# johannes-graeter/limo

Measured on NVIDIA H100. Metric: BA windows/s (30 KF, 3k LM, 40k obs), higher is better.
Workload: dtype f64

## Files before the change

### limo_b200/csrc/kba_api.cu

```cuda
#include <algorithm>
#include <atomic>
#include <chrono>
#include <cstdio>
#include <cstdlib>
#include <cstring>
#include <string>
#include <thread>
#include <vector>

#include <cuda_runtime.h>

#include "kba_b200.h"
#include "kba_kernels.h"

using namespace kba;

static thread_local std::string g_last_error;
static thread_local bool g_force_host_pack = false;
static int fail(int code, const std::string& msg) {
    g_last_error = msg;
    return code;
}
#define CU(call)                                                                                              \
    do {                                                                                                      \
// ... 603 lines not shown
        int max_chunks = 1;
        for (auto& d : b->desc_h) max_chunks = std::max(max_chunks, d.n_chunks);
        int p = std::min(16, (6 * h->sm_count + n_windows * pairs - 1) / (n_windows * pairs));
        b->lc.small_syrk = (max_rows <= 184);
        if (b->lc.small_syrk) p = (h->sm_count + n_windows - 1) / n_windows;
        bd.p_split = std::max(1, std::min(p, max_chunks));
        const char* fe = std::getenv("KBA_FUSED");
        bd.fused = (b->lc.small_syrk && bd.max_kf <= kFusedMaxKf && !(fe && std::atoi(fe) == 0)) ? 1 : 0;
        if (const char* pe = std::getenv("KBA_P_SPLIT")) { if (std::atoi(pe) > 0) p = std::atoi(pe); }
        if (bd.fused) bd.p_split = std::max(1, std::min(p, max_groups));
        else if (std::getenv("KBA_P_SPLIT")) bd.p_split = std::max(1, std::min(p, max_chunks));
        b->lc.fused_slots = (max_rows_free <= 176) ? 6 : 7;
    }
    bd.cost_parts = std::max((bd.max_obs + 255) / 256, (bd.max_obs / 16 + bd.max_lm / 32 + 4 + 7) / 8);
    { const char* le = std::getenv("KBA_LINEARIZE"); b->lc.lin_fused = !(le && std::atoi(le) == 0); }
    { const char* le = std::getenv("KBA_LIN_BLOCKS"); if (le && std::atoi(le) == 3) b->lc.lin_blocks = 3; }
    { const char* le = std::getenv("KBA_LIN_GRID"); if (le) b->lc.lin_grid = std::max(-1, std::atoi(le)); }
    { const char* le = std::getenv("KBA_BS_GRID"); if (le) b->lc.bs_grid = std::max(-1, std::atoi(le)); }
    {
        auto knob = [](const char* name, int dflt) { const char* e = std::getenv(name); return e ? std::atoi(e) : dflt; };
        bd.eval_tiles_jac = std::max(1, knob("KBA_EVAL_TILES_JAC", 8));
        bd.eval_tiles_cost = std::max(1, knob("KBA_EVAL_TILES_COST", 8));
        bd.eval_min_blocks = knob("KBA_EVAL_MIN_BLOCKS", 2);
        bd.eval_cs = knob("KBA_EVAL_CS", 0);
        bd.solve_row_major = knob("KBA_SOLVE_ROW_MAJOR", 0);
        bd.solve_tiled = (nr_cap_max <= 192 && !bd.solve_row_major) ? 1 : 0;
        const int split_dflt = (!bd.solve_tiled && n_windows <= 16) ? std::max(1, std::min(32, h->sm_count / n_windows)) : 0;
        bd.solve_split = bd.solve_tiled ? 0 : knob("KBA_SOLVE_SPLIT", split_dflt);
    }
    bd.bs_parts = (bd.max_lm + 15) / 16;
    {
// ... 242 lines not shown
    launch_reset(b->bd, lc, s);
    const int rounds_max = 7;
    const int max_passes = rounds_max * (3 * opt->trim_solver_iterations + 4) + opt->final_solver_iterations + 8;
    const auto t0 = std::chrono::steady_clock::now();
    int check_every = 4;
    bool timed_out = false, poll_pending = false;
    int gmode = solve_graph_mode();
    if (h->kernel_timing || launch_check_enabled() || s == nullptr || b->sg.unusable) gmode = 0;
    const bool lockstep = b->bd.sharded != 0;
    if (lockstep) gmode = (gmode && shard_graph_enabled() && b->solves_done > 0) ? 1 : 0;
    if (gmode) {
        std::vector<unsigned char> key;
        key.reserve(sizeof(BatchDev) + sizeof(SolveParams) + 64);
        key_append(key, b->bd); key_append(key, sp); key_append(key, gmode); key_append(key, max_passes); key_append(key, s);
        key_append(key, lc.nr_cap_max); key_append(key, lc.max_rank); key_append(key, (int)lc.small_syrk); key_append(key, (int)lc.lin_fused);
        key_append(key, lc.lin_blocks); key_append(key, lc.fused_slots); key_append(key, lc.xchg.user);
        key_append(key, lc.lin_grid); key_append(key, lc.bs_grid);
        if (!(b->sg.exec && b->sg.key == key) && !build_solve_graph(b, sp, lc, gmode, max_passes, check_every, key)) gmode = 0;
    }
    if (gmode == 2) {
        CU(cudaMemsetAsync(b->loop_pass.d, 0, sizeof(int), s));
        CU(cudaGraphLaunch(b->sg.exec, s));
        CU(b->loop_pass.download(s));
        CU(cudaEventRecord(b->ev_b, s));
        CU(b->jac_obs.download(s));
        CU(wait_stream(h));
        CU(cudaGetLastError());
        CU(cudaEventElapsedTime(&b->last_solve_ms, b->ev_a, b->ev_b));
        h->counters.jacobian_obs += (long long)b->jac_obs.h[0];
        add_pass_counters(h->counters, b->sg.per_pass, b->loop_pass.h[0]);
        h->counters.launches_total += b->loop_pass.h[0];
// ... 531 lines not shown
```

### limo_b200/csrc/kba_device.cuh

```cuda
#pragma once
#include <cstdint>
#include <cuda_runtime.h>

namespace kba {

constexpr int kMaxKf = 128;
constexpr int kMaxCam = 8;
constexpr int kPoseStride = 12;
constexpr int kCamStride = 16;
constexpr int kIterLogCap = 160;
constexpr int kFusedMaxKf = 32;

struct WinDesc {
    int n_kf, n_cam, n_lm, n_obs, n_gp;
    int kf_off, cam_off, lm_off, obs_off, gp_off;
    int chunk_off, n_chunks;
    int grp_off, n_groups;
    int scale_kf0, scale_kf1;
    double scale_weight, scale_value;
    double plane_reg_weight;
    int plane_dist_fixed, landmarks_fixed;
    int speed_kf, pad0;
    double speed_weight, speed_dt;
    double speed_v_before[3];
// ... 191 lines not shown
        o[2] = q0 * p[2] - q1 * p[3] + q2 * p[0] + q3 * p[1];
        o[3] = q0 * p[3] + q1 * p[2] - q2 * p[1] + q3 * p[0];
    } else {
        o[0] = p[0]; o[1] = p[1]; o[2] = p[2]; o[3] = p[3];
    }
    o[4] = p[4] + d[3]; o[5] = p[5] + d[4]; o[6] = p[6] + d[5];
}

template <typename T, bool kCost = true>
__device__ inline void cauchy(T b, T w, T s, T& half_rho, T& sqrt_rho1) {
    const T sum = T(1) + s / b;
    half_rho = kCost ? T(0.5) * w * b * log(sum) : T(0);
    sqrt_rho1 = sqrt(w / sum);
}

template <typename T, bool kJac, bool kCost = true>
__device__ inline bool eval_observation(const T* __restrict__ pose, const T* __restrict__ cam, const T p[3], T u, T v,
                                        T d, T wt, T b_repr, T b_depth, T r[3], T jp[18], T jl[9], T& half_rho_sum,
                                        T raw[2]) {
    const T a0 = pose[0] * p[0] + pose[1] * p[1] + pose[2] * p[2];
    const T a1 = pose[3] * p[0] + pose[4] * p[1] + pose[5] * p[2];
    const T a2 = pose[6] * p[0] + pose[7] * p[1] + pose[8] * p[2];
    const T x0 = a0 + pose[9], x1 = a1 + pose[10], x2 = a2 + pose[11];
    const T c0 = cam[0] * x0 + cam[1] * x1 + cam[2] * x2 + cam[9];
    const T c1 = cam[3] * x0 + cam[4] * x1 + cam[5] * x2 + cam[10];
    const T c2 = cam[6] * x0 + cam[7] * x1 + cam[8] * x2 + cam[11];
    if (!(fabs(c2) >= T(0.01))) return false;
    const T f = cam[12], iz = T(1) / c2;
    const T xn = c0 * iz, yn = c1 * iz;
    const T ru = f * xn + cam[13] - u, rv = f * yn + cam[14] - v;
    const T s = ru * ru + rv * rv;
    T hr, sq;
    cauchy<T, kCost>(b_repr, wt, s, hr, sq);
    half_rho_sum = hr;
    raw[0] = sqrt(s);
    raw[1] = T(-1);
    r[0] = sq * ru; r[1] = sq * rv; r[2] = T(0);
    T sqd = T(0), rd = T(0);
    const bool has_d = d > T(0);
    if (has_d) {
        rd = c2 - d;
        T hrd;
        cauchy<T, kCost>(b_depth, wt, rd * rd, hrd, sqd);
        half_rho_sum += hrd;
        raw[1] = fabs(rd);
        r[2] = sqd * rd;
    }
    if (kJac) {
        const T fz = f * iz * sq;
        T m[3][3];
#pragma unroll
        for (int c = 0; c < 3; ++c) {
            m[0][c] = fz * (cam[c] - xn * cam[6 + c]);
            m[1][c] = fz * (cam[3 + c] - yn * cam[6 + c]);
            m[2][c] = sqd * cam[6 + c];
        }
#pragma unroll
        for (int i = 0; i < 3; ++i) {
            jp[6 * i + 0] = T(-2) * (m[i][1] * a2 - m[i][2] * a1);
            jp[6 * i + 1] = T(-2) * (m[i][2] * a0 - m[i][0] * a2);
            jp[6 * i + 2] = T(-2) * (m[i][0] * a1 - m[i][1] * a0);
            jp[6 * i + 3] = m[i][0];
            jp[6 * i + 4] = m[i][1];
            jp[6 * i + 5] = m[i][2];
#pragma unroll
            for (int c = 0; c < 3; ++c) jl[3 * i + c] = m[i][0] * pose[c] + m[i][1] * pose[3 + c] + m[i][2] * pose[6 + c];
        }
    }
    return true;
}

template <typename T, bool kCs>
__device__ __forceinline__ void lin_store(T* p, T v) {
    if (kCs) __stcs(p, v); else *p = v;
}
template <typename T, bool kJl = true, bool kCs = false>
__device__ inline bool eval_observation_store(const T* __restrict__ pose, const T* __restrict__ cam, const T p[3], T u,
                                              T v, T d, T wt, T b_repr, T b_depth, T* __restrict__ res,
                                              T* __restrict__ jp, T* __restrict__ jl, size_t stride, bool write_jp,
                                              T& half_rho_sum) {
    const T a0 = pose[0] * p[0] + pose[1] * p[1] + pose[2] * p[2];
// ... 127 lines not shown
```

### limo_b200/csrc/kba_kernels.cu

```cuda
#include "kba_device.cuh"
#include "kba_kernels.h"
#include "kba_regularisers.cuh"
#include "kba_prep.cuh"
#include "kba_linearize.cuh"

#include <cfloat>
#include <cstdio>
#include <cstdlib>
#include <cmath>
#include <type_traits>

namespace kba {

constexpr int kBeginThreads = 1024;
__global__ void __launch_bounds__(kBeginThreads) k_solve_begin(BatchDev bd, SolveParams sp) {
    const int w = blockIdx.x;
    WinState& st = bd.state[w];
    if (st.phase != PH_SOLVE_BEGIN) return;
    const WinDesc wd = bd.desc[w];
    __shared__ int s_has[kMaxKf];
    __shared__ int s_plane[kMaxKf];
    __shared__ int s_cnt[3];
    __shared__ int s_tile_chunk[513];
    for (int k = threadIdx.x; k < wd.n_kf; k += blockDim.x) { s_has[k] = 0; s_plane[k] = 0; }
// ... 365 lines not shown
        (kJac ? bd.gp_cost_x : bd.gp_cost_c)[w] = s;
    }
}
template __global__ void k_gp_eval<true>(BatchDev, SolveParams);
template __global__ void k_gp_eval<false>(BatchDev, SolveParams);

__global__ void __launch_bounds__(256, 2) k_pose_hessian(BatchDev bd, SolveParams sp) {
    const int w = blockIdx.y, k = blockIdx.x;
    const WinState& st = bd.state[w];
    if (st.phase != PH_ITERATE || !st.need_linearize) return;
    const WinDesc& wd = bd.desc[w];
    if (k >= wd.n_kf || bd.off_pose[wd.kf_off + k] < 0) return;
    __shared__ double s_pose[kPoseStride];
    __shared__ double s_cam[kMaxCam * kCamStride];
    __shared__ double s_red[8][27];
    if (threadIdx.x == 0) {
        const double* p = bd.pose[st.cur] + 7 * (size_t)(wd.kf_off + k);
        double R[9];
        quat_to_rot<double>(p, R);
        for (int i = 0; i < 9; ++i) s_pose[i] = R[i];
        s_pose[9] = p[4]; s_pose[10] = p[5]; s_pose[11] = p[6];
    }
    for (int i = threadIdx.x; i < wd.n_cam * kCamStride; i += blockDim.x) s_cam[i] = bd.cam[(size_t)wd.cam_off * kCamStride + i];
    __syncthreads();
    double acc[27];
#pragma unroll
    for (int q = 0; q < 27; ++q) acc[q] = 0.0;
    const int* kp = bd.kf_ptr + wd.kf_off + w;
    const int e0 = kp[k], e1 = kp[k + 1];
    const double* __restrict__ lm_buf = bd.lm[st.cur];
    const size_t ob = (size_t)wd.obs_off;
    int e = e0 + threadIdx.x;
    int idx_b = (e < e1) ? bd.pm_lm[ob + e] : -1;
    int idx_a = (e + (int)blockDim.x < e1) ? bd.pm_lm[ob + e + blockDim.x] : -1;
    int L = -1, cam = 0;
    float u = 0.f, v = 0.f, d = 0.f;
    double p0 = 0, p1 = 0, p2 = 0, wgt = 0;
    unsigned char act = 0;
    if (idx_b >= 0) {
        L = wd.lm_off + idx_b;
        cam = bd.pm_cam[ob + e]; u = bd.pm_u[ob + e]; v = bd.pm_v[ob + e]; d = bd.pm_d[ob + e];
        p0 = lm_buf[3 * (size_t)L]; p1 = lm_buf[3 * (size_t)L + 1]; p2 = lm_buf[3 * (size_t)L + 2];
        wgt = bd.lm_weight[L]; act = bd.lm_active[L];
    }
#pragma unroll 1
    for (; e < e1; e += blockDim.x) {
        const int en = e + blockDim.x;
        int Ln = -1, camn = 0;
        float un = 0.f, vn = 0.f, dn = 0.f;
        double q0 = 0, q1 = 0, q2 = 0, wn = 0;
        unsigned char actn = 0;
        if (idx_a >= 0) {
            Ln = wd.lm_off + idx_a;
            camn = bd.pm_cam[ob + en]; un = bd.pm_u[ob + en]; vn = bd.pm_v[ob + en]; dn = bd.pm_d[ob + en];
            q0 = lm_buf[3 * (size_t)Ln]; q1 = lm_buf[3 * (size_t)Ln + 1]; q2 = lm_buf[3 * (size_t)Ln + 2];
            wn = bd.lm_weight[Ln]; actn = bd.lm_active[Ln];
        }
        idx_a = (en + (int)blockDim.x < e1) ? bd.pm_lm[ob + en + blockDim.x] : -1;
        if (act) {
            const double p[3] = {p0, p1, p2};
            double r[3], jp[18], jl[9], raw[2], hr;
            if (eval_observation<double, true, false>(s_pose, s_cam + kCamStride * cam, p, (double)u, (double)v, (double)d,
                                                      wgt, sp.reprojection_thres * sp.reprojection_thres,
                                                      sp.depth_thres * sp.depth_thres, r, jp, jl, hr, raw)) {
                int q = 0;
#pragma unroll
                for (int a = 0; a < 6; ++a)
#pragma unroll
                    for (int b = a; b < 6; ++b) {
                        acc[q] += jp[a] * jp[b] + jp[6 + a] * jp[6 + b] + jp[12 + a] * jp[12 + b];
                        ++q;
                    }
#pragma unroll
                for (int a = 0; a < 6; ++a) acc[21 + a] += jp[a] * r[0] + jp[6 + a] * r[1] + jp[12 + a] * r[2];
            }
        }
        L = Ln; cam = camn; u = un; v = vn; d = dn; p0 = q0; p1 = q1; p2 = q2; wgt = wn; act = actn;
    }
#pragma unroll
    for (int q = 0; q < 27; ++q) {
        const double v = warp_sum(acc[q]);
        if ((threadIdx.x & 31) == 0) s_red[threadIdx.x >> 5][q] = v;
    }
    __syncthreads();
    if (threadIdx.x < 27) {
        double s = 0.0;
        for (int q = 0; q < 8; ++q) s += s_red[q][threadIdx.x];
        bd.bkf[(size_t)(wd.kf_off + k) * 27 + threadIdx.x] = s;
    }
}

constexpr int kLC = 32;
constexpr int kKC = 3 * kLC;

__device__ __forceinline__ int gp_row(const BatchDev& bd, const WinDesc& wd, int k, int r) {
    if (r < 6) { const int o = bd.off_pose[wd.kf_off + k]; return o < 0 ? -1 : o + r; }
// ... 1591 lines not shown
        e = cudaFuncSetAttribute(k_reduced_solve<true>, cudaFuncAttributeMaxDynamicSharedMemorySize,
                                 (int)solve_tiled_smem(nr_cap_max));
        if (e != cudaSuccess) return e;
        hi_tiled[dev] = nr_cap_max;
    }
    if (nr_cap_max > hi_rows[dev]) {
        e = cudaFuncSetAttribute(k_chol_trail, cudaFuncAttributeMaxDynamicSharedMemorySize, (int)trail_smem(nr_cap_max));
        if (e != cudaSuccess) return e;
        e = cudaFuncSetAttribute(k_reduced_solve<false>, cudaFuncAttributeMaxDynamicSharedMemorySize, (int)solve_smem(nr_cap_max));
        if (e != cudaSuccess) return e;
        hi_rows[dev] = nr_cap_max;
    }
    return cudaSuccess;
}

static int strided_grid(int cfg, int n_units, int num, int den, int n_win, int sm_count) {
    if (cfg == 0) return n_units;
    if (cfg > 0) return cfg < n_units ? cfg : n_units;
    const int g = (n_units * num + den - 1) / den;
    return ((long long)g * n_win >= 8LL * 2 * sm_count && g >= 1) ? g : n_units;
}

void launch_reset(const BatchDev& bd, const LaunchCfg& lc, cudaStream_t s) {
    k_reset_state<<<bd.n_win, 256, 0, s>>>(bd, lc.rounds_override, lc.min_landmarks_for_trimming, lc.num_rounds_option); LCHK("k_reset_state");
}

int launch_pass(const BatchDev& bd, const SolveParams& sp, const LaunchCfg& lc, Counters* cnt, cudaStream_t s) {
    const int B = bd.n_win;
    const dim3 g_obs((bd.max_obs + 255) / 256, B);
    const dim3 g_lm((bd.max_lm + 63) / 64, B);
    if (!bd.fused) k_panel_zero<<<dim3(64, B), 256, 0, s>>>(bd);
    LCHK("k_panel_zero");
    k_solve_begin<<<B, kBeginThreads, 0, s>>>(bd, sp); LCHK("k_solve_begin");
    const bool timed = lc.time_jacobian && lc.ev_pool && *lc.ev_used + 2 <= lc.ev_cap;
    const bool lin1 = bd.lin1 != 0;
    if (lin1) {
        if (bd.tot_gp > 0) k_gp_eval<true><<<B, 256, 0, s>>>(bd, sp);
        LCHK("k_gp_eval");
        if (timed) cudaEventRecord(lc.ev_pool[(*lc.ev_used)++], s);
        const int n_units = (lin_tile_bound(bd.max_obs, bd.max_lm) + kLinWarps - 1) / kLinWarps;
        const dim3 g_lin(strided_grid(lc.lin_grid, n_units, 1, 5, B, lc.sm_count), B);
        if ((int)g_lin.x < n_units) k_linearize<2, true><<<g_lin, kLinThreads, 0, s>>>(bd, sp, n_units);
        else if (lc.lin_blocks == 3) k_linearize<3, false><<<g_lin, kLinThreads, 0, s>>>(bd, sp, n_units);
        else k_linearize<2, false><<<g_lin, kLinThreads, 0, s>>>(bd, sp, n_units);
        LCHK("k_linearize");
        if (timed) cudaEventRecord(lc.ev_pool[(*lc.ev_used)++], s);
        k_pose_hessian<<<dim3(bd.max_kf, B), 256, 0, s>>>(bd, sp); LCHK("k_pose_hessian");
    } else {
        if (timed) cudaEventRecord(lc.ev_pool[(*lc.ev_used)++], s);
        launch_eval_obs<true>(bd, sp, s);
        if (timed) cudaEventRecord(lc.ev_pool[(*lc.ev_used)++], s);
        if (bd.tot_gp > 0) k_gp_eval<true><<<B, 256, 0, s>>>(bd, sp);
        LCHK("k_gp_eval");
        k_pose_hessian<<<dim3(bd.max_kf, B), 256, 0, s>>>(bd, sp); LCHK("k_pose_hessian");
    }
    if (bd.fused) {
        if (!lin1) {
            k_landmark_reduce<true><<<dim3((bd.max_lm + 15) / 16, B), 256, 0, s>>>(bd, sp); LCHK("k_landmark_reduce");
            k_obs_v2<<<g_obs, 256, 0, s>>>(bd); LCHK("k_obs_v2");
// ... 35 lines not shown
        k_reduced_solve<true><<<B, 512, solve_tiled_smem(lc.nr_cap_max), s>>>(bc, sp, 0); LCHK("k_reduced_solve");
    } else if (!bd.solve_split) {
        k_reduced_solve<false><<<B, 512, solve_smem(lc.nr_cap_max), s>>>(bc, sp, 0); LCHK("k_reduced_solve");
    } else {
        k_reduced_solve<false><<<B, 512, solve_smem(lc.nr_cap_max), s>>>(bc, sp, 1); LCHK("k_reduced_solve");
        const int strips = (lc.nr_cap_max + 7) / 8;
        for (int kb = 0; kb < lc.nr_cap_max; kb += kNB) {
            k_chol_diag<<<B, 32, 0, s>>>(bc, kb); LCHK("k_chol_diag");
            k_chol_panel<<<dim3((strips + 15) / 16, B), 512, 0, s>>>(bc, kb); LCHK("k_chol_panel");
            k_chol_trail<<<dim3(bd.solve_split, B), 512, trail_smem(lc.nr_cap_max), s>>>(bc, kb); LCHK("k_chol_trail");
        }
        k_reduced_solve<false><<<B, 512, solve_smem(lc.nr_cap_max), s>>>(bc, sp, 2); LCHK("k_reduced_solve");
    }
    if (bd.fused) {
        const int n_units = (bd.max_lm + 15) / 16;
        const int gx = strided_grid(lc.bs_grid, n_units, 1, 3, B, lc.sm_count);
        if (gx < n_units) k_backsub_v<true><<<dim3(gx, B), 256, 0, s>>>(bd, n_units);
        else k_backsub_v<false><<<dim3(n_units, B), 256, 0, s>>>(bd, n_units);
    }
    else k_backsub<<<dim3((bd.max_lm + 15) / 16, B), 256, 0, s>>>(bd);
    LCHK("k_backsub");
    launch_eval_obs<false>(bd, sp, s);
    if (bd.tot_gp > 0) k_gp_eval<false><<<B, 256, 0, s>>>(bd, sp);
    LCHK("k_gp_eval");
    if (bd.sharded) {
        k_shard_scalars<<<1, 256, 0, s>>>(bd); LCHK("k_shard_scalars");
        if (int rc = lc.xchg.allreduce(lc.xchg.user, bd.xs, bd.xs, 16 + bd.shard_world, 0, s)) return rc;
    }
    k_lm_update<<<(B * 32 + 127) / 128, 128, 0, s>>>(bd, sp); LCHK("k_lm_update");
    k_trim_eval<<<g_lm, 256, 0, s>>>(bd, sp); LCHK("k_trim_eval");
    if (bd.sharded) {
// ... 71 lines not shown
```

### limo_b200/csrc/kba_kernels.h

```cpp
#pragma once
#include <cuda_runtime.h>

#include "kba_device.cuh"

namespace kba {

int launch_check_enabled();
void launch_check_report(const char* kernel, cudaError_t e);
#define LCHK(name)                                                                       \
    do {                                                                                 \
        if (kba::launch_check_enabled()) {                                               \
            const cudaError_t lchk_e_ = cudaGetLastError();                              \
            if (lchk_e_ != cudaSuccess) kba::launch_check_report(name, lchk_e_);         \
        }                                                                                \
    } while (0)

struct Counters {
    long long launches_total = 0;
    long long launches_jacobian = 0, launches_prep = 0, launches_schur = 0, launches_solve = 0, launches_backsub = 0,
              launches_cost = 0, launches_update = 0, launches_trim = 0;
    double ms_jacobian = 0.0;
    long long jacobian_obs = 0;
};

struct Exchange {
    int (*allreduce)(void* user, const double* send, double* recv, long long count, int op, cudaStream_t s) = nullptr;
    void* user = nullptr;
    int rank = 0, world = 1;
};

struct LaunchCfg {
    int nr_cap_max = 64;
    int sm_count = 132;
    int max_rank = 0;
    bool small_syrk = false;
    bool lin_fused = true;
    int lin_blocks = 2;
    int lin_grid = -1;
    int bs_grid = -1;
    int fused_slots = 6;
    int rounds_override = -1, min_landmarks_for_trimming = 100, num_rounds_option = 1;
    bool time_jacobian = false;
    cudaEvent_t* ev_pool = nullptr;
    int ev_cap = 0;
    int* ev_used = nullptr;
    Exchange xchg;
    struct WinDescHost { int nr_cap = 0, n_kf = 0; } shard_win;
};

struct PackRaw {
    const int* lm_ptr = nullptr;
    const int* obs_kf = nullptr;
// ... 51 lines not shown
```

### limo_b200/csrc/kba_linearize.cuh

```cuda
#pragma once
#include "kba_device.cuh"

namespace kba {

constexpr int kLinThreads = 256;
constexpr int kLinWarps = kLinThreads / 32;

__host__ __device__ __forceinline__ int lin_tile_bound(int n_obs, int n_lm) { return n_obs / 16 + n_lm / 32 + 4; }
__device__ __forceinline__ size_t lin_tile_offset(const WinDesc& wd, int w) {
    return (size_t)(wd.obs_off / 16) + (size_t)(wd.lm_off / 32) + 4 * (size_t)w;
}

__device__ inline void build_lin_tiles(const BatchDev& bd, const WinDesc& wd, WinState& st, int w, int* s_chunk ) {
    const int* lm_ptr = bd.lm_ptr + wd.lm_off + w;
    int2* tiles = bd.lin_tile + lin_tile_offset(wd, w);
    const int per = max(64, (wd.n_lm + 511) / 512);
    const int n_chunks = (wd.n_lm + per - 1) / per;
    for (int pass = 0; pass < 2; ++pass) {
        for (int c = threadIdx.x; c < n_chunks; c += blockDim.x) {
            const int j0 = c * per, j1 = min(wd.n_lm, j0 + per);
            int n = 0, t_start = 0, t_cnt = 0;
            int2* out = tiles + (pass ? s_chunk[c] : 0);
            int o0 = lm_ptr[j0];
            for (int j = j0; j < j1; ++j) {
// ... 11 lines not shown
        __syncthreads();
        if (!pass) {
            if (threadIdx.x == 0) {
                int acc = 0;
                for (int c = 0; c < n_chunks; ++c) { const int t = s_chunk[c]; s_chunk[c] = acc; acc += t; }
                if (acc > lin_tile_bound(wd.n_obs, wd.n_lm)) acc = 0;
                st.n_lin_tiles = acc;
                s_chunk[512] = acc;
            }
            __syncthreads();
            if (s_chunk[512] == 0) return;
        }
    }
}

template <int kMinBlocks, bool kLoop>
__global__ void __launch_bounds__(kLinThreads, kMinBlocks) k_linearize(BatchDev bd, SolveParams sp, int n_units) {
    const int w = blockIdx.y;
    WinState& st = bd.state[w];
    if (st.phase != PH_ITERATE) return;
    const WinDesc& wd = bd.desc[w];
    const int n_tiles = st.n_lin_tiles;
    const bool lin = st.need_linearize != 0;
    const bool want_cost = lin && st.iter0;
    if (wd.landmarks_fixed && !want_cost) return;
    const int tid = threadIdx.x, lane = tid & 31, warp = tid >> 5;
    __shared__ __align__(16) double s_pose[kFusedMaxKf * kPoseStride];
    __shared__ __align__(16) double s_cam[kMaxCam * kCamStride];
    __shared__ __align__(8) uint64_t s_bar;
    __shared__ double s_cg[kLinWarps][9][33];
    __shared__ double s_red[kLinWarps];
    __shared__ int s_cnt[kLinWarps];
    bool staged = false;
    for (int unit = blockIdx.x; unit < n_units; unit += gridDim.x) {
    if (unit * kLinWarps >= n_tiles) {
        if (tid == 0 && want_cost) bd.cost_part_x[(size_t)w * bd.cost_parts + unit] = 0.0;
        if constexpr (!kLoop) return;
        continue;
    }
    const size_t base = (size_t)wd.obs_off;
    const int* lm_ptr = bd.lm_ptr + wd.lm_off + w;
    const int t = unit * kLinWarps + warp;
    int2 tile = make_int2(0, 0);
    if (t < n_tiles) tile = bd.lin_tile[lin_tile_offset(wd, w) + t];
    const bool have = lane < tile.y;
    const int o = tile.x + lane;
    int j = 0, kf = 0, cam = 0, row0 = -1, p0 = 0, p1 = 0;
    float mu = 0.f, mv = 0.f, md = 0.f;
    double p[3] = {0, 0, 0}, wgt = 0.0;
    bool act = false;
    if (have) {
        const size_t oo = base + o;
        j = bd.obs_lm[oo];
        kf = bd.obs_kf[oo]; cam = bd.obs_cam[oo]; row0 = bd.obs_row[oo];
        mu = bd.obs_u[oo]; mv = bd.obs_v[oo]; md = bd.obs_d[oo];
        p0 = lm_ptr[j]; p1 = lm_ptr[j + 1];
        act = bd.lm_active[wd.lm_off + j] != 0;
        const double* lmp = bd.lm[st.cur] + 3 * (size_t)(wd.lm_off + j);
        p[0] = lmp[0]; p[1] = lmp[1]; p[2] = lmp[2];
        wgt = bd.lm_weight[wd.lm_off + j];
    }
    const int L = wd.lm_off + j;
    if (!staged) {
        stage_window_bulk(wd, bd.rt[st.cur], bd.cam, s_pose, s_cam, &s_bar);
        staged = true;
    }
    double jp[18];
    bool ok = true;
    double hr = 0.0;
    double cg[9] = {0, 0, 0, 0, 0, 0, 0, 0, 0};
    if (act) {
        double r[3], jl[9], raw[2];
        const double* ps = s_pose + kPoseStride * kf;
        const double* cs_ = s_cam + kCamStride * cam;
        const double br = sp.reprojection_thres * sp.reprojection_thres, bdp = sp.depth_thres * sp.depth_thres;
        if (want_cost) ok = eval_observation<double, true, true>(ps, cs_, p, (double)mu, (double)mv, (double)md, wgt, br, bdp, r, jp, jl, hr, raw);
        else ok = eval_observation<double, true, false>(ps, cs_, p, (double)mu, (double)mv, (double)md, wgt, br, bdp, r, jp, jl, hr, raw);
        if (ok) {
            cg[0] = jl[0] * jl[0] + jl[3] * jl[3] + jl[6] * jl[6];
            cg[1] = jl[0] * jl[1] + jl[3] * jl[4] + jl[6] * jl[7];
            cg[2] = jl[0] * jl[2] + jl[3] * jl[5] + jl[6] * jl[8];
            cg[3] = jl[1] * jl[1] + jl[4] * jl[4] + jl[7] * jl[7];
            cg[4] = jl[1] * jl[2] + jl[4] * jl[5] + jl[7] * jl[8];
            cg[5] = jl[2] * jl[2] + jl[5] * jl[5] + jl[8] * jl[8];
#pragma unroll
            for (int c = 0; c < 3; ++c) cg[6 + c] = jl[c] * r[0] + jl[3 + c] * r[1] + jl[6 + c] * r[2];
        } else {
            hr = 0.0;
            if (lin) st.eval_failed = 1;
        }
    }
    {
        const double cs = warp_sum(hr);
        const int dn = __reduce_add_sync(0xffffffffu, (act && ok) ? 1 : 0);
        if (lane == 0) { s_red[warp] = cs; s_cnt[warp] = dn; }
    }
    if (!wd.landmarks_fixed) {
        double (*sw)[33] = s_cg[warp];
#pragma unroll
        for (int q = 0; q < 9; ++q) sw[q][lane] = cg[q];
        const int seg0 = p0 - tile.x;
        const int klen = p1 - p0;
        double tt_ld[3] = {0.0, 0.0, 0.0};
        if (act && !st.iter0) {
#pragma unroll
            for (int e = 0; e < 3; ++e) tt_ld[e] = bd.lm_scale[3 * (size_t)L + e];
        }
        __syncwarp();
        if (have) {
            for (int q = lane - seg0; q < 9; q += klen) {
                double sacc = 0.0;
                for (int l = seg0; l < seg0 + klen; ++l) sacc += sw[q][l];
                sw[q][seg0] = sacc;
            }
        }
        __syncwarp();
        if (act) {
            double c[6], g[3];
#pragma unroll
            for (int q = 0; q < 6; ++q) c[q] = sw[q][seg0];
#pragma unroll
            for (int q = 0; q < 3; ++q) g[q] = sw[6 + q][seg0];
            const bool first = lane == seg0;
            const int gl = (wd.n_gp > 0) ? bd.gp_of_lm[L] : -1;
            const size_t TG = (size_t)bd.tot_gp, G = (size_t)wd.gp_off + (gl >= 0 ? gl : 0);
            double gjl[3] = {0, 0, 0};
            if (gl >= 0) {
                gjl[0] = bd.gp_lin[11 * TG + G]; gjl[1] = bd.gp_lin[12 * TG + G]; gjl[2] = bd.gp_lin[13 * TG + G];
                const double gr = bd.gp_lin[G];
                c[0] += gjl[0] * gjl[0]; c[1] += gjl[0] * gjl[1]; c[2] += gjl[0] * gjl[2];
                c[3] += gjl[1] * gjl[1]; c[4] += gjl[1] * gjl[2]; c[5] += gjl[2] * gjl[2];
                g[0] += gjl[0] * gr; g[1] += gjl[1] * gr; g[2] += gjl[2] * gr;
// ... 30 lines not shown
                    for (int e = 0; e < 3; ++e) {
                        bd.lm_g[3 * (size_t)L + e] = g[e];
                        bd.lm_lambda[3 * (size_t)L + e] = lam[e];
                        if (st.iter0) bd.lm_scale[3 * (size_t)L + e] = tt[e];
                    }
                    if (gl >= 0) {
                        for (int rr = 0; rr < 10; ++rr) {
                            const double jf_ = bd.gp_lin[(1 + rr) * TG + G];
                            const double e0 = jf_ * gjl[0], e1 = jf_ * gjl[1], e2 = jf_ * gjl[2];
                            bd.vgp[(3 * rr + 0) * TG + G] = e0 * i00;
                            bd.vgp[(3 * rr + 1) * TG + G] = e0 * i10 + e1 * i11;
                            bd.vgp[(3 * rr + 2) * TG + G] = e0 * i20 + e1 * i21 + e2 * i22;
                        }
                    }
                }
                if (ok && row0 >= 0) {
                    const double* R = s_pose + kPoseStride * kf;
                    double wm[9];
#pragma unroll
                    for (int r = 0; r < 3; ++r) {
                        const double m0 = jp[6 * r + 3], m1 = jp[6 * r + 4], m2 = jp[6 * r + 5];
                        const double l0 = m0 * R[0] + m1 * R[3] + m2 * R[6], l1 = m0 * R[1] + m1 * R[4] + m2 * R[7], l2 = m0 * R[2] + m1 * R[5] + m2 * R[8];
                        wm[3 * r + 0] = l0 * i00;
                        wm[3 * r + 1] = l0 * i10 + l1 * i11;
                        wm[3 * r + 2] = l0 * i20 + l1 * i21 + l2 * i22;
                    }
#pragma unroll
                    for (int cc = 0; cc < 3; ++cc) {
                        double2* out = reinterpret_cast<double2*>(bd.vobs + vobs_index(base, p0, p1, o, cc));
#pragma unroll
                        for (int h = 0; h < 3; ++h) {
                            const int r0 = 2 * h, r1 = 2 * h + 1;
                            out[h] = make_double2(jp[r0] * wm[cc] + jp[6 + r0] * wm[3 + cc] + jp[12 + r0] * wm[6 + cc],
                                                  jp[r1] * wm[cc] + jp[6 + r1] * wm[3 + cc] + jp[12 + r1] * wm[6 + cc]);
                        }
                    }
                }
            }
        }
    }
    __syncthreads();
    if (tid == 0) {
        double s = 0.0;
        int cnt = 0;
        for (int q = 0; q < kLinWarps; ++q) { s += s_red[q]; cnt += s_cnt[q]; }
        if (want_cost) bd.cost_part_x[(size_t)w * bd.cost_parts + unit] = s;
        if (cnt) atomicAdd(bd.jac_obs, (unsigned long long)cnt);
    }
    if constexpr (!kLoop) break;
    if (unit + (int)gridDim.x < n_units) __syncthreads();
    }
}

}
```

Baseline: 1211.

## Factor observation Jacobians via projection Gram matrix in linearize and pose Hessian

```diff
diff --git a/limo_b200/csrc/kba_api.cu b/limo_b200/csrc/kba_api.cu
--- a/limo_b200/csrc/kba_api.cu
+++ b/limo_b200/csrc/kba_api.cu
@@ -641,7 +641,6 @@
     }
     bd.cost_parts = std::max((bd.max_obs + 255) / 256, (bd.max_obs / 16 + bd.max_lm / 32 + 4 + 7) / 8);
     { const char* le = std::getenv("KBA_LINEARIZE"); b->lc.lin_fused = !(le && std::atoi(le) == 0); }
-    { const char* le = std::getenv("KBA_LIN_BLOCKS"); if (le && std::atoi(le) == 3) b->lc.lin_blocks = 3; }
     { const char* le = std::getenv("KBA_LIN_GRID"); if (le) b->lc.lin_grid = std::max(-1, std::atoi(le)); }
     { const char* le = std::getenv("KBA_BS_GRID"); if (le) b->lc.bs_grid = std::max(-1, std::atoi(le)); }
     {
@@ -914,7 +913,7 @@
         key.reserve(sizeof(BatchDev) + sizeof(SolveParams) + 64);
         key_append(key, b->bd); key_append(key, sp); key_append(key, gmode); key_append(key, max_passes); key_append(key, s);
         key_append(key, lc.nr_cap_max); key_append(key, lc.max_rank); key_append(key, (int)lc.small_syrk); key_append(key, (int)lc.lin_fused);
-        key_append(key, lc.lin_blocks); key_append(key, lc.fused_slots); key_append(key, lc.xchg.user);
+        key_append(key, lc.fused_slots); key_append(key, lc.xchg.user);
         key_append(key, lc.lin_grid); key_append(key, lc.bs_grid);
         if (!(b->sg.exec && b->sg.key == key) && !build_solve_graph(b, sp, lc, gmode, max_passes, check_every, key)) gmode = 0;
     }
diff --git a/limo_b200/csrc/kba_device.cuh b/limo_b200/csrc/kba_device.cuh
--- a/limo_b200/csrc/kba_device.cuh
+++ b/limo_b200/csrc/kba_device.cuh
@@ -229,18 +229,20 @@
     sqrt_rho1 = sqrt(w / sum);
 }
 
-template <typename T, bool kJac, bool kCost = true>
-__device__ inline bool eval_observation(const T* __restrict__ pose, const T* __restrict__ cam, const T p[3], T u, T v,
-                                        T d, T wt, T b_repr, T b_depth, T r[3], T jp[18], T jl[9], T& half_rho_sum,
-                                        T raw[2]) {
-    const T a0 = pose[0] * p[0] + pose[1] * p[1] + pose[2] * p[2];
-    const T a1 = pose[3] * p[0] + pose[4] * p[1] + pose[5] * p[2];
-    const T a2 = pose[6] * p[0] + pose[7] * p[1] + pose[8] * p[2];
-    const T x0 = a0 + pose[9], x1 = a1 + pose[10], x2 = a2 + pose[11];
+template <typename T, bool kM, bool kCost = true>
+__device__ __forceinline__ bool eval_factored(const T* __restrict__ pose, const T* __restrict__ cam, const T p[3], T u, T v,
+                                              T d, T wt, T b_repr, T b_depth, T r[3], T m[9], T a[3], T& half_rho_sum,
+                                              T raw[2]) {
+    a[0] = pose[0] * p[0] + pose[1] * p[1] + pose[2] * p[2];
+    a[1] = pose[3] * p[0] + pose[4] * p[1] + pose[5] * p[2];
+    a[2] = pose[6] * p[0] + pose[7] * p[1] + pose[8] * p[2];
+    const T x0 = a[0] + pose[9], x1 = a[1] + pose[10], x2 = a[2] + pose[11];
     const T c0 = cam[0] * x0 + cam[1] * x1 + cam[2] * x2 + cam[9];
     const T c1 = cam[3] * x0 + cam[4] * x1 + cam[5] * x2 + cam[10];
     const T c2 = cam[6] * x0 + cam[7] * x1 + cam[8] * x2 + cam[11];
     if (!(fabs(c2) >= T(0.01))) return false;
+    const bool has_d = d > T(0);
+    const T rd = has_d ? c2 - d : T(0);
     const T f = cam[12], iz = T(1) / c2;
     const T xn = c0 * iz, yn = c1 * iz;
     const T ru = f * xn + cam[13] - u, rv = f * yn + cam[14] - v;
@@ -251,35 +253,57 @@
     raw[0] = sqrt(s);
     raw[1] = T(-1);
     r[0] = sq * ru; r[1] = sq * rv; r[2] = T(0);
-    T sqd = T(0), rd = T(0);
-    const bool has_d = d > T(0);
+    T sqd = T(0);
     if (has_d) {
-        rd = c2 - d;
         T hrd;
         cauchy<T, kCost>(b_depth, wt, rd * rd, hrd, sqd);
         half_rho_sum += hrd;
         raw[1] = fabs(rd);
         r[2] = sqd * rd;
     }
+    if (kM) {
+        const T fz = f * iz * sq;
+#pragma unroll
+        for (int c = 0; c < 3; ++c) {
+            m[c] = fz * (cam[c] - xn * cam[6 + c]);
+            m[3 + c] = fz * (cam[3 + c] - yn * cam[6 + c]);
+            m[6 + c] = sqd * cam[6 + c];
+        }
+    }
+    return true;
+}
+
+__host__ __device__ constexpr int sym3(int i, int j) {
+    return i <= j ? 3 * i + j - i * (i + 1) / 2 : 3 * j + i - j * (j + 1) / 2;
+}
+
+__device__ __forceinline__ void gram_factored(const double m[9], double M[6]) {
+    M[0] = m[0] * m[0] + m[3] * m[3] + m[6] * m[6];
+    M[1] = m[0] * m[1] + m[3] * m[4] + m[6] * m[7];
+    M[2] = m[0] * m[2] + m[3] * m[5] + m[6] * m[8];
+    M[3] = m[1] * m[1] + m[4] * m[4] + m[7] * m[7];
+    M[4] = m[1] * m[2] + m[4] * m[5] + m[7] * m[8];
+    M[5] = m[2] * m[2] + m[5] * m[5] + m[8] * m[8];
+}
+
+template <typename T, bool kJac, bool kCost = true>
+__device__ inline bool eval_observation(const T* __restrict__ pose, const T* __restrict__ cam, const T p[3], T u, T v,
+                                        T d, T wt, T b_repr, T b_depth, T r[3], T jp[18], T jl[9], T& half_rho_sum,
+                                        T raw[2]) {
+    T m[9], a[3];
+    if (!eval_factored<T, kJac, kCost>(pose, cam, p, u, v, d, wt, b_repr, b_depth, r, m, a, half_rho_sum, raw)) return false;
     if (kJac) {
-        const T fz = f * iz * sq;
-        T m[3][3];
-#pragma unroll
-        for (int c = 0; c < 3; ++c) {
-            m[0][c] = fz * (cam[c] - xn * cam[6 + c]);
-            m[1][c] = fz * (cam[3 + c] - yn * cam[6 + c]);
-            m[2][c] = sqd * cam[6 + c];
-        }
 #pragma unroll
         for (int i = 0; i < 3; ++i) {
-            jp[6 * i + 0] = T(-2) * (m[i][1] * a2 - m[i][2] * a1);
-            jp[6 * i + 1] = T(-2) * (m[i][2] * a0 - m[i][0] * a2);
-            jp[6 * i + 2] = T(-2) * (m[i][0] * a1 - m[i][1] * a0);
-            jp[6 * i + 3] = m[i][0];
-            jp[6 * i + 4] = m[i][1];
-            jp[6 * i + 5] = m[i][2];
-#pragma unroll
-            for (int c = 0; c < 3; ++c) jl[3 * i + c] = m[i][0] * pose[c] + m[i][1] * pose[3 + c] + m[i][2] * pose[6 + c];
+            const T* mi = m + 3 * i;
+            jp[6 * i + 0] = T(-2) * (mi[1] * a[2] - mi[2] * a[1]);
+            jp[6 * i + 1] = T(-2) * (mi[2] * a[0] - mi[0] * a[2]);
+            jp[6 * i + 2] = T(-2) * (mi[0] * a[1] - mi[1] * a[0]);
+            jp[6 * i + 3] = mi[0];
+            jp[6 * i + 4] = mi[1];
+            jp[6 * i + 5] = mi[2];
+#pragma unroll
+            for (int c = 0; c < 3; ++c) jl[3 * i + c] = mi[0] * pose[c] + mi[1] * pose[3 + c] + mi[2] * pose[6 + c];
         }
     }
     return true;
diff --git a/limo_b200/csrc/kba_kernels.cu b/limo_b200/csrc/kba_kernels.cu
--- a/limo_b200/csrc/kba_kernels.cu
+++ b/limo_b200/csrc/kba_kernels.cu
@@ -403,7 +403,11 @@
     __shared__ double s_pose[kPoseStride];
     __shared__ double s_cam[kMaxCam * kCamStride];
     __shared__ double s_red[8][27];
+    __shared__ double s_acc[9][256];
+    __shared__ long long s_ob;
+    __shared__ int s_lm_off, s_e1;
     if (threadIdx.x == 0) {
+        s_ob = wd.obs_off; s_lm_off = wd.lm_off; s_e1 = bd.kf_ptr[wd.kf_off + w + k + 1];
         const double* p = bd.pose[st.cur] + 7 * (size_t)(wd.kf_off + k);
         double R[9];
         quat_to_rot<double>(p, R);
@@ -412,9 +416,11 @@
     }
     for (int i = threadIdx.x; i < wd.n_cam * kCamStride; i += blockDim.x) s_cam[i] = bd.cam[(size_t)wd.cam_off * kCamStride + i];
     __syncthreads();
-    double acc[27];
-#pragma unroll
-    for (int q = 0; q < 27; ++q) acc[q] = 0.0;
+    double acc[18];
+#pragma unroll
+    for (int q = 0; q < 18; ++q) acc[q] = 0.0;
+#pragma unroll
+    for (int q = 0; q < 9; ++q) s_acc[q][threadIdx.x] = 0.0;
     const int* kp = bd.kf_ptr + wd.kf_off + w;
     const int e0 = kp[k], e1 = kp[k + 1];
     const double* __restrict__ lm_buf = bd.lm[st.cur];
@@ -433,42 +439,60 @@
         wgt = bd.lm_weight[L]; act = bd.lm_active[L];
     }
 #pragma unroll 1
-    for (; e < e1; e += blockDim.x) {
+    for (; e < s_e1; e += blockDim.x) {
+        asm volatile("" ::: "memory");
+        const size_t obs0 = (size_t)s_ob;
+        const int e_end = s_e1, lm0 = s_lm_off;
         const int en = e + blockDim.x;
         int Ln = -1, camn = 0;
         float un = 0.f, vn = 0.f, dn = 0.f;
         double q0 = 0, q1 = 0, q2 = 0, wn = 0;
         unsigned char actn = 0;
         if (idx_a >= 0) {
-            Ln = wd.lm_off + idx_a;
-            camn = bd.pm_cam[ob + en]; un = bd.pm_u[ob + en]; vn = bd.pm_v[ob + en]; dn = bd.pm_d[ob + en];
+            Ln = lm0 + idx_a;
+            camn = bd.pm_cam[obs0 + en]; un = bd.pm_u[obs0 + en]; vn = bd.pm_v[obs0 + en]; dn = bd.pm_d[obs0 + en];
             q0 = lm_buf[3 * (size_t)Ln]; q1 = lm_buf[3 * (size_t)Ln + 1]; q2 = lm_buf[3 * (size_t)Ln + 2];
             wn = bd.lm_weight[Ln]; actn = bd.lm_active[Ln];
         }
-        idx_a = (en + (int)blockDim.x < e1) ? bd.pm_lm[ob + en + blockDim.x] : -1;
+        idx_a = (en + (int)blockDim.x < e_end) ? bd.pm_lm[obs0 + en + blockDim.x] : -1;
         if (act) {
             const double p[3] = {p0, p1, p2};
-            double r[3], jp[18], jl[9], raw[2], hr;
-            if (eval_observation<double, true, false>(s_pose, s_cam + kCamStride * cam, p, (double)u, (double)v, (double)d,
-                                                      wgt, sp.reprojection_thres * sp.reprojection_thres,
-                                                      sp.depth_thres * sp.depth_thres, r, jp, jl, hr, raw)) {
-                int q = 0;
-#pragma unroll
-                for (int a = 0; a < 6; ++a)
-#pragma unroll
-                    for (int b = a; b < 6; ++b) {
-                        acc[q] += jp[a] * jp[b] + jp[6 + a] * jp[6 + b] + jp[12 + a] * jp[12 + b];
-                        ++q;
+            double r[3], m[9], a[3], raw[2], hr;
+            if (eval_factored<double, true, false>(s_pose, s_cam + kCamStride * cam, p, (double)u, (double)v, (double)d,
+                                                   wgt, sp.reprojection_thres * sp.reprojection_thres,
+                                                   sp.depth_thres * sp.depth_thres, r, m, a, hr, raw)) {
+                double mm[6], h[3];
+                gram_factored(m, mm);
+#pragma unroll
+                for (int c = 0; c < 3; ++c) h[c] = m[c] * r[0] + m[3 + c] * r[1] + m[6 + c] * r[2];
+#pragma unroll
+                for (int i = 0; i < 3; ++i) {
+                    const int i1 = (i + 1) % 3, i2 = (i + 2) % 3;
+                    double pr[3];
+#pragma unroll
+                    for (int c = 0; c < 3; ++c) pr[c] = 2.0 * (a[i1] * mm[sym3(i2, c)] - a[i2] * mm[sym3(i1, c)]);
+                    const int qd = 6 * i - i * (i - 1) / 2;
+#pragma unroll
+                    for (int j = i; j < 3; ++j) {
+                        const int j1 = (j + 1) % 3, j2 = (j + 2) % 3;
+                        acc[qd + j - i] += 2.0 * (a[j1] * pr[j2] - a[j2] * pr[j1]);
                     }
 #pragma unroll
-                for (int a = 0; a < 6; ++a) acc[21 + a] += jp[a] * r[0] + jp[6 + a] * r[1] + jp[12 + a] * r[2];
+                    for (int c = 0; c < 3; ++c) acc[qd + 3 - i + c] += pr[c];
+                    acc[15 + i] += 2.0 * (a[i1] * h[i2] - a[i2] * h[i1]);
+                }
+#pragma unroll
+                for (int q = 0; q < 6; ++q) s_acc[q][threadIdx.x] += mm[q];
+#pragma unroll
+                for (int c = 0; c < 3; ++c) s_acc[6 + c][threadIdx.x] += h[c];
             }
         }
         L = Ln; cam = camn; u = un; v = vn; d = dn; p0 = q0; p1 = q1; p2 = q2; wgt = wn; act = actn;
     }
 #pragma unroll
     for (int q = 0; q < 27; ++q) {
-        const double v = warp_sum(acc[q]);
+        const double t = q < 15 ? acc[q] : q < 21 ? s_acc[q - 15][threadIdx.x] : q < 24 ? acc[q - 6] : s_acc[q - 18][threadIdx.x];
+        const double v = warp_sum(t);
         if ((threadIdx.x & 31) == 0) s_red[threadIdx.x >> 5][q] = v;
     }
     __syncthreads();
@@ -2090,11 +2114,11 @@
     return cudaSuccess;
 }
 
-static int strided_grid(int cfg, int n_units, int num, int den, int n_win, int sm_count) {
+static int strided_grid(int cfg, int n_units, int num, int den, int n_win, int sm_count, int ctas_per_sm, int waves) {
     if (cfg == 0) return n_units;
     if (cfg > 0) return cfg < n_units ? cfg : n_units;
     const int g = (n_units * num + den - 1) / den;
-    return ((long long)g * n_win >= 8LL * 2 * sm_count && g >= 1) ? g : n_units;
+    return ((long long)g * n_win >= (long long)waves * ctas_per_sm * sm_count && g >= 1) ? g : n_units;
 }
 
 void launch_reset(const BatchDev& bd, const LaunchCfg& lc, cudaStream_t s) {
@@ -2115,10 +2139,9 @@
         LCHK("k_gp_eval");
         if (timed) cudaEventRecord(lc.ev_pool[(*lc.ev_used)++], s);
         const int n_units = (lin_tile_bound(bd.max_obs, bd.max_lm) + kLinWarps - 1) / kLinWarps;
-        const dim3 g_lin(strided_grid(lc.lin_grid, n_units, 1, 5, B, lc.sm_count), B);
-        if ((int)g_lin.x < n_units) k_linearize<2, true><<<g_lin, kLinThreads, 0, s>>>(bd, sp, n_units);
-        else if (lc.lin_blocks == 3) k_linearize<3, false><<<g_lin, kLinThreads, 0, s>>>(bd, sp, n_units);
-        else k_linearize<2, false><<<g_lin, kLinThreads, 0, s>>>(bd, sp, n_units);
+        const dim3 g_lin(strided_grid(lc.lin_grid, n_units, 1, 8, B, lc.sm_count, kLinMinBlocks, 6), B);
+        if ((int)g_lin.x < n_units) k_linearize<true><<<g_lin, kLinThreads, 0, s>>>(bd, sp, n_units);
+        else k_linearize<false><<<g_lin, kLinThreads, 0, s>>>(bd, sp, n_units);
         LCHK("k_linearize");
         if (timed) cudaEventRecord(lc.ev_pool[(*lc.ev_used)++], s);
         k_pose_hessian<<<dim3(bd.max_kf, B), 256, 0, s>>>(bd, sp); LCHK("k_pose_hessian");
@@ -2184,7 +2207,7 @@
     }
     if (bd.fused) {
         const int n_units = (bd.max_lm + 15) / 16;
-        const int gx = strided_grid(lc.bs_grid, n_units, 1, 3, B, lc.sm_count);
+        const int gx = strided_grid(lc.bs_grid, n_units, 1, 3, B, lc.sm_count, 2, 8);
         if (gx < n_units) k_backsub_v<true><<<dim3(gx, B), 256, 0, s>>>(bd, n_units);
         else k_backsub_v<false><<<dim3(n_units, B), 256, 0, s>>>(bd, n_units);
     }
diff --git a/limo_b200/csrc/kba_kernels.h b/limo_b200/csrc/kba_kernels.h
--- a/limo_b200/csrc/kba_kernels.h
+++ b/limo_b200/csrc/kba_kernels.h
@@ -35,7 +35,6 @@
     int max_rank = 0;
     bool small_syrk = false;
     bool lin_fused = true;
-    int lin_blocks = 2;
     int lin_grid = -1;
     int bs_grid = -1;
     int fused_slots = 6;
diff --git a/limo_b200/csrc/kba_linearize.cuh b/limo_b200/csrc/kba_linearize.cuh
--- a/limo_b200/csrc/kba_linearize.cuh
+++ b/limo_b200/csrc/kba_linearize.cuh
@@ -1,4 +1,5 @@
 #pragma once
+#include <type_traits>
 #include "kba_device.cuh"
 
 namespace kba {
@@ -49,27 +50,35 @@
     }
 }
 
-template <int kMinBlocks, bool kLoop>
-__global__ void __launch_bounds__(kLinThreads, kMinBlocks) k_linearize(BatchDev bd, SolveParams sp, int n_units) {
+constexpr int kLinMinBlocks = 3;
+constexpr size_t kLinStaticSmem = sizeof(double) * (kFusedMaxKf * kPoseStride + kMaxCam * kCamStride + kLinWarps * 9 * 33 +
+                                                    kLinWarps * 32 * 9 + kLinWarps) +
+                                  sizeof(int) * (kLinWarps * 6 * 32 + kLinWarps) + sizeof(uint64_t);
+static_assert(kLinStaticSmem <= 48 * 1024, "k_linearize: static shared memory over 48 KB");
+template <bool kLoop>
+__global__ void __launch_bounds__(kLinThreads, kLinMinBlocks) k_linearize(BatchDev bd, SolveParams sp, int n_units) {
     const int w = blockIdx.y;
     WinState& st = bd.state[w];
     if (st.phase != PH_ITERATE) return;
     const WinDesc& wd = bd.desc[w];
-    const int n_tiles = st.n_lin_tiles;
-    const bool lin = st.need_linearize != 0;
-    const bool want_cost = lin && st.iter0;
-    if (wd.landmarks_fixed && !want_cost) return;
+    const volatile WinState& vst = st;
+    const auto n_tiles = [&] { return vst.n_lin_tiles; };
+    const auto lin = [&] { return vst.need_linearize != 0; };
+    const auto want_cost = [&] { return vst.need_linearize != 0 && vst.iter0 != 0; };
+    if (wd.landmarks_fixed && !want_cost()) return;
     const int tid = threadIdx.x, lane = tid & 31, warp = tid >> 5;
     __shared__ __align__(16) double s_pose[kFusedMaxKf * kPoseStride];
     __shared__ __align__(16) double s_cam[kMaxCam * kCamStride];
     __shared__ __align__(8) uint64_t s_bar;
     __shared__ double s_cg[kLinWarps][9][33];
+    __shared__ double s_ma[kLinWarps][32][9];
+    __shared__ int s_ix[kLinWarps][6][32];
     __shared__ double s_red[kLinWarps];
     __shared__ int s_cnt[kLinWarps];
-    bool staged = false;
     for (int unit = blockIdx.x; unit < n_units; unit += gridDim.x) {
-    if (unit * kLinWarps >= n_tiles) {
-        if (tid == 0 && want_cost) bd.cost_part_x[(size_t)w * bd.cost_parts + unit] = 0.0;
+    asm volatile("" ::: "memory");
+    if (unit * kLinWarps >= n_tiles()) {
+        if (tid == 0 && want_cost()) bd.cost_part_x[(size_t)w * bd.cost_parts + unit] = 0.0;
         if constexpr (!kLoop) return;
         continue;
     }
@@ -77,7 +86,7 @@
     const int* lm_ptr = bd.lm_ptr + wd.lm_off + w;
     const int t = unit * kLinWarps + warp;
     int2 tile = make_int2(0, 0);
-    if (t < n_tiles) tile = bd.lin_tile[lin_tile_offset(wd, w) + t];
+    if (t < n_tiles()) tile = bd.lin_tile[lin_tile_offset(wd, w) + t];
     const bool have = lane < tile.y;
     const int o = tile.x + lane;
     int j = 0, kf = 0, cam = 0, row0 = -1, p0 = 0, p1 = 0;
@@ -95,23 +104,35 @@
         p[0] = lmp[0]; p[1] = lmp[1]; p[2] = lmp[2];
         wgt = bd.lm_weight[wd.lm_off + j];
     }
-    const int L = wd.lm_off + j;
-    if (!staged) {
-        stage_window_bulk(wd, bd.rt[st.cur], bd.cam, s_pose, s_cam, &s_bar);
-        staged = true;
-    }
-    double jp[18];
-    bool ok = true;
+    int (*six)[32] = s_ix[warp];
+    if (unit == (int)blockIdx.x) stage_window_bulk(wd, bd.rt[st.cur], bd.cam, s_pose, s_cam, &s_bar);
+    six[0][lane] = kf; six[1][lane] = row0; six[2][lane] = wd.obs_off + p0; six[3][lane] = p1 - p0; six[4][lane] = wd.lm_off + j;
+    six[5][lane] = have ? 1 | (act ? 2 : 0) | ((p0 - tile.x) << 2) : 0;
+    double* sma = s_ma[warp][lane];
+    bool ok = false;
     double hr = 0.0;
     double cg[9] = {0, 0, 0, 0, 0, 0, 0, 0, 0};
     if (act) {
-        double r[3], jl[9], raw[2];
-        const double* ps = s_pose + kPoseStride * kf;
-        const double* cs_ = s_cam + kCamStride * cam;
-        const double br = sp.reprojection_thres * sp.reprojection_thres, bdp = sp.depth_thres * sp.depth_thres;
-        if (want_cost) ok = eval_observation<double, true, true>(ps, cs_, p, (double)mu, (double)mv, (double)md, wgt, br, bdp, r, jp, jl, hr, raw);
-        else ok = eval_observation<double, true, false>(ps, cs_, p, (double)mu, (double)mv, (double)md, wgt, br, bdp, r, jp, jl, hr, raw);
-        if (ok) {
+        const auto evaluate = [&](auto with_cost) {
+            double r[3], m[9], raw[2];
+            const double br = sp.reprojection_thres * sp.reprojection_thres, bdp = sp.depth_thres * sp.depth_thres;
+            ok = eval_factored<double, true, decltype(with_cost)::value>(s_pose + kPoseStride * kf, s_cam + kCamStride * cam, p,
+                                                                          (double)mu, (double)mv, (double)md, wgt, br, bdp, r, m,
+                                                                          sma + 6, hr, raw);
+            if (!ok) return;
+            {
+                unsigned t;
+                asm volatile("mov.u32 %0, %%tid.x;" : "=r"(t));
+                s_ix[t >> 5][5][t & 31] |= 128;
+            }
+            gram_factored(m, sma);
+            const double* R = s_pose + kPoseStride * reinterpret_cast<volatile int*>(six[0])[lane];
+            double jl[9];
+#pragma unroll
+            for (int i = 0; i < 3; ++i) {
+#pragma unroll
+                for (int c = 0; c < 3; ++c) jl[3 * i + c] = m[3 * i] * R[c] + m[3 * i + 1] * R[3 + c] + m[3 * i + 2] * R[6 + c];
+            }
             cg[0] = jl[0] * jl[0] + jl[3] * jl[3] + jl[6] * jl[6];
             cg[1] = jl[0] * jl[1] + jl[3] * jl[4] + jl[6] * jl[7];
             cg[2] = jl[0] * jl[2] + jl[3] * jl[5] + jl[6] * jl[8];
@@ -120,29 +141,34 @@
             cg[5] = jl[2] * jl[2] + jl[5] * jl[5] + jl[8] * jl[8];
 #pragma unroll
             for (int c = 0; c < 3; ++c) cg[6 + c] = jl[c] * r[0] + jl[3 + c] * r[1] + jl[6 + c] * r[2];
-        } else {
+        };
+        if (want_cost()) evaluate(std::true_type{});
+        else evaluate(std::false_type{});
+        if (!ok) {
             hr = 0.0;
-            if (lin) st.eval_failed = 1;
+            if (lin()) st.eval_failed = 1;
         }
     }
     {
         const double cs = warp_sum(hr);
-        const int dn = __reduce_add_sync(0xffffffffu, (act && ok) ? 1 : 0);
+        const int dn = __reduce_add_sync(0xffffffffu, ok ? 1 : 0);
         if (lane == 0) { s_red[warp] = cs; s_cnt[warp] = dn; }
     }
     if (!wd.landmarks_fixed) {
         double (*sw)[33] = s_cg[warp];
 #pragma unroll
         for (int q = 0; q < 9; ++q) sw[q][lane] = cg[q];
-        const int seg0 = p0 - tile.x;
-        const int klen = p1 - p0;
+        __syncwarp();
+        const int L = six[4][lane];
+        const bool in_tile = six[5][lane] & 1, active = six[5][lane] & 2;
+        const int seg0 = (six[5][lane] >> 2) & 31;
+        const int klen = six[3][lane];
         double tt_ld[3] = {0.0, 0.0, 0.0};
-        if (act && !st.iter0) {
+        if (active && !st.iter0) {
 #pragma unroll
             for (int e = 0; e < 3; ++e) tt_ld[e] = bd.lm_scale[3 * (size_t)L + e];
         }
-        __syncwarp();
-        if (have) {
+        if (in_tile) {
             for (int q = lane - seg0; q < 9; q += klen) {
                 double sacc = 0.0;
                 for (int l = seg0; l < seg0 + klen; ++l) sacc += sw[q][l];
@@ -150,7 +176,7 @@
             }
         }
         __syncwarp();
-        if (act) {
+        if (active) {
             double c[6], g[3];
 #pragma unroll
             for (int q = 0; q < 6; ++q) c[q] = sw[q][seg0];
@@ -211,12 +237,13 @@
                         }
                     }
                 }
-                if (ok && row0 >= 0) {
-                    const double* R = s_pose + kPoseStride * kf;
+                if ((six[5][lane] & 128) && six[1][lane] >= 0) {
+                    const double* R = s_pose + kPoseStride * six[0][lane];
+                    const int g0 = six[2][lane];
                     double wm[9];
 #pragma unroll
                     for (int r = 0; r < 3; ++r) {
-                        const double m0 = jp[6 * r + 3], m1 = jp[6 * r + 4], m2 = jp[6 * r + 5];
+                        const double m0 = sma[sym3(r, 0)], m1 = sma[sym3(r, 1)], m2 = sma[sym3(r, 2)];
                         const double l0 = m0 * R[0] + m1 * R[3] + m2 * R[6], l1 = m0 * R[1] + m1 * R[4] + m2 * R[7], l2 = m0 * R[2] + m1 * R[5] + m2 * R[8];
                         wm[3 * r + 0] = l0 * i00;
                         wm[3 * r + 1] = l0 * i10 + l1 * i11;
@@ -224,13 +251,12 @@
                     }
 #pragma unroll
                     for (int cc = 0; cc < 3; ++cc) {
-                        double2* out = reinterpret_cast<double2*>(bd.vobs + vobs_index(base, p0, p1, o, cc));
-#pragma unroll
-                        for (int h = 0; h < 3; ++h) {
-                            const int r0 = 2 * h, r1 = 2 * h + 1;
-                            out[h] = make_double2(jp[r0] * wm[cc] + jp[6 + r0] * wm[3 + cc] + jp[12 + r0] * wm[6 + cc],
-                                                  jp[r1] * wm[cc] + jp[6 + r1] * wm[3 + cc] + jp[12 + r1] * wm[6 + cc]);
-                        }
+                        double2* out = reinterpret_cast<double2*>(bd.vobs + vobs_index(0, g0, g0 + klen, g0 + lane - seg0, cc));
+                        const double w0 = wm[cc], w1 = wm[3 + cc], w2 = wm[6 + cc];
+                        const double a0 = sma[6], a1 = sma[7], a2 = sma[8];
+                        out[0] = make_double2(2.0 * (a1 * w2 - a2 * w1), 2.0 * (a2 * w0 - a0 * w2));
+                        out[1] = make_double2(2.0 * (a0 * w1 - a1 * w0), w0);
+                        out[2] = make_double2(w1, w2);
                     }
                 }
             }
@@ -241,7 +267,7 @@
         double s = 0.0;
         int cnt = 0;
         for (int q = 0; q < kLinWarps; ++q) { s += s_red[q]; cnt += s_cnt[q]; }
-        if (want_cost) bd.cost_part_x[(size_t)w * bd.cost_parts + unit] = s;
+        if (want_cost()) bd.cost_part_x[(size_t)w * bd.cost_parts + unit] = s;
         if (cnt) atomicAdd(bd.jac_obs, (unsigned long long)cnt);
     }
     if constexpr (!kLoop) break;
```

After: 1330 (median of 6 runs). 1.1x the previous value.
